# famoreno/stereo-vo

Hardware: AMD Instinct MI355X
Metric: stereo pairs/sec @1280×960 (higher is better)
Workload: dtype u8/f64

## Files before the change

### stereo_vo_amd/csrc/k_detect.hip

```cpp
#include <algorithm>
#include "svo_device.h"
#include "svo_kernels.h"
#include "../../include/svo_orb_tables.h"

__constant__ int c_umax[16];
__device__ __attribute__((aligned(16))) float4 g_brief_patf[SVO_BRIEF_NPAIRS];
__device__ __attribute__((aligned(16))) uint4 g_blur_gh[3 * 64], g_blur_gv[3 * 64];
#define SVO_DISC_E 256
__device__ uint32_t g_disc_m[SVO_DISC_E], g_disc_x[SVO_DISC_E];
#define DP_REACH SVO_BRIEF_REACH
#define DP_BW (2 * DP_REACH + 1)
#define DP_RW (DP_BW + 6)
#define DP_X0 (DP_REACH + 5)

hipError_t svo_upload_tables()
{
    hipError_t e = hipMemcpyToSymbol(HIP_SYMBOL(c_umax), svo_umax, sizeof(svo_umax));
    if (e != hipSuccess) return e;
    {
        static float4 pf[SVO_BRIEF_NPAIRS];
        for (int i = 0; i < SVO_BRIEF_NPAIRS; i++) pf[i] = make_float4((float)svo_brief_pat[i][0], (float)svo_brief_pat[i][2], (float)svo_brief_pat[i][1], (float)svo_brief_pat[i][3]);
        e = hipMemcpyToSymbol(HIP_SYMBOL(g_brief_patf), pf, sizeof(pf));
        if (e != hipSuccess) return e;
    }
// ... 346 lines not shown
#pragma unroll
        for (int g = 0; g < FT_ROWS; g++) {
            const uint32_t Cp = col[(g + 3) * (FT_LW / 4)], C = cc[g + 3], Cn = col[(g + 3) * (FT_LW / 4) + 2], N = cc[g], S = cc[g + 6];
            const uint32_t Eo = __builtin_amdgcn_alignbyte(Cn, C, 3), Wo = __builtin_amdgcn_alignbyte(C, Cp, 1);
            const uint32_t Ee = __builtin_amdgcn_alignbyte(Cn, C, 2);
            pe[g] = quick_half(C << 8, N << 8, Ee, S << 8, Cp, t2h);
            po[g] = quick_half(C, N, Eo, S, Wo, t2h);
        }
    }
    auto entry_of = [&](int b) -> int { return e_base + ((b & 7) << 6) + (b >> 3); };
    uint32_t m_left = 0;
    {
        const uint32_t one2 = 0x00010001u;
        uint32_t me = 0, mo = 0;
#pragma unroll
        for (int g = FT_ROWS - 1; g >= 0; g--) {
            uint32_t fe, fo;
            asm("v_pk_min_u16 %0, %1, %2" : "=v"(fe) : "v"(pe[g]), "s"(one2));
            asm("v_pk_min_u16 %0, %1, %2" : "=v"(fo) : "v"(po[g]), "s"(one2));
            if (g == FT_ROWS - 1) { me = fe; mo = fo; }
            else {
                asm("v_lshl_or_b32 %0, %1, 1, %2" : "=v"(me) : "v"(me), "v"(fe));
                asm("v_lshl_or_b32 %0, %1, 1, %2" : "=v"(mo) : "v"(mo), "v"(fo));
            }
        }
        uint32_t m = me | (mo << 8);
        const int cnt = __popc(m), inc = wave_inclusive_scan(cnt);
        const int total = __builtin_amdgcn_readlane(inc, 63);
        if (total) {
            unsigned wbase = 0;
            if ((tid & 63) == 0) wbase = atomicAdd(&s_count, (unsigned)total);
            unsigned idx = (unsigned)__builtin_amdgcn_readfirstlane((int)wbase) + (unsigned)(inc - cnt);
            while (m && idx < FT_LIST_CAP) {
                const int b = __builtin_ctz(m); m &= m - 1;
                list[idx++] = (unsigned short)entry_of(b);
            }
            m_left = m;
        }
    }
    __syncthreads();
    const int ns_all = (int)s_count, ns = min(ns_all, FT_LIST_CAP);
    const bool overflow = ns_all > FT_LIST_CAP;
    if (c.debug_mode == 2) return;
    auto win_off = [&](int e) -> int { return (e >> 6) * FT_LW + (e & 63) + (3 * FT_LW + 4); };
    for (int i = tid; i < ns; i += FT_NT) {
        const int e = list[i];
        score[e] = (uint8_t)fast_score_lds(tile, win_off(e), th_fast);
    }
    if (__builtin_expect(overflow, 0)) {
        for (uint32_t m = m_left; m; m &= m - 1) {
            const int e = entry_of(__builtin_ctz(m));
            score[e] = (uint8_t)fast_score_lds(tile, win_off(e), th_fast);
        }
    }
    __syncthreads();
    if (c.debug_mode == 3) return;
    auto nms_round = [&](bool has, int e) {
        bool keep = false; uint32_t key = 0;
        if (has) {
            const int r = e >> 6, q = e & 63;
            const int nb = e - FT_SP - 1; int nbm = nb; asm volatile("" : "+v"(nbm));
            const int v = score[nbm + FT_SP + 1];
            const int n0 = score[nb], n1 = score[nbm + 1], n2 = score[nb + 2], n3 = score[nb + FT_SP], n4 = score[nb + FT_SP + 2];
            const int n5 = score[nb + 2 * FT_SP], n6 = score[nbm + 2 * FT_SP + 1], n7 = score[nb + 2 * FT_SP + 2];
            const int mx = max(max(max(n0, n1), max(n2, n3)), max(max(n4, n5), max(n6, n7)));
            const int x = x0 - 1 + q, y = y0 - 1 + r;
            keep = (v > mx) & (r >= 1) & (r <= FT_H) & (q >= 1) & (q <= FT_W) & (x < gw - SVO_EDGE) & (y < gh - SVO_EDGE);
            key = ((uint32_t)v << 24) | (0xFFFFFFu - (uint32_t)(y * gw + x));
        }
        const unsigned long long m = __ballot(keep);
        if (m) {
            unsigned b2 = 0;
            const int leader = __ffsll((long long)m) - 1;
            if ((tid & 63) == leader) b2 = atomicAdd(&s_nout, (unsigned)__popcll(m));
            b2 = __shfl(b2, leader, 64);
            if (keep) out_keys[b2 + __popcll(m & ((1ull << (tid & 63)) - 1ull))] = key;
        }
    };
    for (int base = 0; base < ns; base += FT_NT) {
        const int i = base + tid;
        nms_round(i < ns, i < ns ? (int)list[i] : 0);
    }
    if (__builtin_expect(overflow, 0)) {
        uint32_t m = m_left;
        while (__ballot(m != 0)) {
            const bool has = m != 0;
            const int e = has ? entry_of(__builtin_ctz(m)) : 0;
            m &= m - 1;
            nms_round(has, e);
        }
    }
    __syncthreads();
    if (tid < 64) {
        const unsigned nout = s_nout;
        if (nout != 0 && c.debug_mode != 4) {
            const LevelGeom& g = c.lv[level];
            unsigned gbase = 0;
            if (tid == 0) gbase = atomicAdd(&c.cand_cnt[(img * SVO_MAX_LEVELS + level) * SVO_CNT_STRIDE], nout);
            gbase = __shfl(gbase, 0, 64);
            uint32_t* dst = c.cand_keys + (long long)img * c.cand_total + g.cand_off;
            for (unsigned i = tid; i < nout; i += 64) {
                if (gbase + i < (unsigned)g.cand_cap) dst[gbase + i] = out_keys[i];
                else raise_detect_status(c, img >> 1, SVO_ST_CAND_OVERFLOW);
            }
        }
    }
}

__global__ void __launch_bounds__(FT_NT) __attribute__((amdgpu_waves_per_eu(8, 8))) k_fast(DevCtx c)
{
    SVO_TL_SCOPE(c, TL_FAST, 0);
    __shared__ FastSmem sm;
    const uint32_t slot = blockIdx.x >> 3;
    const uint32_t work = c.debug_mode == 8 ? blockIdx.x : (((slot / FT_CHUNK) * 8 + (blockIdx.x & 7)) * FT_CHUNK + slot % FT_CHUNK);
    const int img = (int)fastdiv(work, c.div_tiles), tile_id = (int)work - img * c.n_tiles;
    if (img >= c.n_img) return;
    const uint4 e = c.fast_tiles[tile_id];
    const uint4 tha = ((const uint4*)(c.fast_th_used + img * SVO_MAX_LEVELS))[0], thb = ((const uint4*)(c.fast_th_used + img * SVO_MAX_LEVELS))[1];
    const uint8_t* base0 = c.img0[img];
    const int level = (int)(e.z & 0xFFu);
    const uint32_t thv[8] = { tha.x, tha.y, tha.z, tha.w, thb.x, thb.y, thb.z, thb.w };
    uint32_t th = thv[0];
#pragma unroll
    for (int l = 1; l < SVO_MAX_LEVELS; l++) th = level == l ? thv[l] : th;
    const uint8_t* src = level == 0 ? base0 : c.pyr + (long long)img * c.pyr_bytes + e.w;
    const int pitch = level == 0 ? c.img0_pitch : (int)(e.z >> 8);
    fast_tile(c, sm, img, level, src, pitch, (int)(e.y & 0xFFFFu), (int)(e.y >> 16), (int)(e.x & 0xFFFFu), (int)(e.x >> 16), (int)th);
}

__global__ void __launch_bounds__(FT_NT) k_fast_redo(DevCtx c)
{
    SVO_TL_SCOPE(c, TL_FAST, 1);
    __shared__ FastSmem sm;
    const unsigned n = *c.redo_n;
    if (n == 0) return;
    int first = (int)blockIdx.x;
    for (unsigned e = 0; e < n; e++) {
        const uint32_t il = c.redo_list[e];
        const int img = (int)(il / SVO_MAX_LEVELS), level = (int)(il % SVO_MAX_LEVELS);
        const int nt = c.lv[level].tiles_x * c.lv[level].tiles_y;
        int t = first;
        int pitch; const uint8_t* src = level_ptr(c, img, level, pitch);
        const int tx = c.lv[level].tiles_x, gw = c.lv[level].w, gh = c.lv[level].h;
        for (; t < nt; t += (int)gridDim.x) {
            const int by = t / tx, bx = t - by * tx;
            fast_tile(c, sm, img, level, src, pitch, gw, gh, SVO_EDGE + bx * FT_W, SVO_EDGE + by * FT_H, c.fast_th);
            __syncthreads();
        }
        first = t - nt;
    }
}


__device__ __forceinline__ float harris_at(const uint8_t* img, int pitch, int x, int y)
{
    int a = 0, b = 0, cc = 0;
    for (int dy = -3; dy <= 3; dy++) {
        const uint8_t* pm = img + (long long)(y + dy - 1) * pitch + x, *p0 = pm + pitch, *pp = p0 + pitch;
#pragma unroll
        for (int dx = -3; dx <= 3; dx++) {
            const int Ix = ((int)p0[dx + 1] - (int)p0[dx - 1]) * 2 + ((int)pm[dx + 1] - (int)pm[dx - 1]) + ((int)pp[dx + 1] - (int)pp[dx - 1]);
            const int Iy = ((int)pp[dx] - (int)pm[dx]) * 2 + ((int)pp[dx - 1] - (int)pm[dx - 1]) + ((int)pp[dx + 1] - (int)pm[dx + 1]);
            a += Ix * Ix; b += Iy * Iy; cc += Ix * Iy;
        }
    }
    const float s = 1.0f / (4.0f * 7.0f * 255.0f);
    const float s4 = s * s * s * s;
    const float fa = (float)a, fb = (float)b, fc = (float)cc;
    const float tr = fa + fb;
    return (fa * fb - fc * fc - 0.04f * tr * tr) * s4;
}

__device__ __forceinline__ float harris_at_dw(const uint8_t* img, int pitch, int x, int y)
{
    const int xa = (x - 4) & ~3, o = (x - 4) & 3;
    int px[9][9];
#pragma unroll
    for (int r = 0; r < 9; r++) {
        const uint3 pw = *(const uint3*)(img + (long long)(y - 4 + r) * pitch + xa);
        const uint32_t w0 = pw.x, w1 = pw.y, w2 = pw.z;
        const uint32_t A = __builtin_amdgcn_alignbyte(w1, w0, o), B = __builtin_amdgcn_alignbyte(w2, w1, o), C = w2 >> (8 * o);
#pragma unroll
        for (int k = 0; k < 4; k++) { px[r][k] = (A >> (8 * k)) & 0xFF; px[r][4 + k] = (B >> (8 * k)) & 0xFF; }
        px[r][8] = C & 0xFF;
    }
    int a = 0, b = 0, cc = 0;
#pragma unroll
    for (int r = 1; r < 8; r++) {
#pragma unroll
        for (int q = 1; q < 8; q++) {
            const int Ix = (px[r][q + 1] - px[r][q - 1]) * 2 + (px[r - 1][q + 1] - px[r - 1][q - 1]) + (px[r + 1][q + 1] - px[r + 1][q - 1]);
            const int Iy = (px[r + 1][q] - px[r - 1][q]) * 2 + (px[r + 1][q - 1] - px[r - 1][q - 1]) + (px[r + 1][q + 1] - px[r - 1][q + 1]);
            a += __mul24(Ix, Ix); b += __mul24(Iy, Iy); cc += __mul24(Ix, Iy);
        }
    }
    const float s = 1.0f / (4.0f * 7.0f * 255.0f);
    const float s4 = s * s * s * s;
    const float fa = (float)a, fb = (float)b, fc = (float)cc;
    const float tr = fa + fb;
    return (fa * fb - fc * fc - 0.04f * tr * tr) * s4;
}

template <int SEL_MAX>
__device__ __forceinline__ int select_block(const DevCtx& c, int redo_pass, int img, int level, unsigned long long* keys, uint32_t* sel, unsigned* hist, int* scan_s, unsigned* sv)
{
    constexpr int SEL_TIE_MAX = 2 * SEL_MAX;
    unsigned& s_prefix = sv[0]; unsigned& s_need = sv[1]; unsigned& s_sel = sv[2]; unsigned& s_tie = sv[3]; unsigned& s_ntie = sv[4];
    const LevelGeom& g = c.lv[level];
    const int tid = threadIdx.x;
    const int il = img * SVO_MAX_LEVELS + level;
    if (redo_pass && !c.redo_flag[il]) return 0;
    unsigned nc = c.cand_cnt[il * SVO_CNT_STRIDE];
    if (nc > (unsigned)g.cand_cap) nc = g.cand_cap;
    const unsigned K = min(nc, (unsigned)(2 * g.quota));
    const uint32_t th_used = c.fast_th_used[il], th_base = (uint32_t)c.fast_th;
    if (!redo_pass && g.quota > 0 && th_used > th_base && nc < (unsigned)(2 * g.quota)) {
        if (tid == 0) {
            c.redo_flag[il] = 1; c.redo_list[atomicAdd(c.redo_n, 1u)] = (uint32_t)il;
            atomicAdd(c.redo_n + 1, 1u);
            c.cand_cnt[il * SVO_CNT_STRIDE] = 0; c.fast_th_used[il] = th_base; c.fast_th_dyn[il] = 0;
        }
        return 0;
    }
    if (K == 0 || g.quota <= 0) { if (tid == 0) { c.lvl_n[il] = 0; c.sel_n[il] = 0; c.fast_th_dyn[il] = 0; } return 0; }
    const uint32_t* ck = c.cand_keys + (long long)img * c.cand_total + g.cand_off;
    uint32_t* tie = (uint32_t*)keys;
    for (int i = tid; i < 256; i += blockDim.x) hist[i] = 0;
    if (tid == 0) { s_sel = 0; s_tie = 0; }
    __syncthreads();
    for (unsigned base = tid; base < nc; base += 8 * 512) {
        uint32_t k[8];
#pragma unroll
        for (int u = 0; u < 8; u++) { const unsigned i = base + u * 512; k[u] = i < nc ? ck[i] : 0u; }
#pragma unroll
        for (int u = 0; u < 8; u++) if (base + u * 512 < nc) atomicAdd(&hist[k[u] >> 24], 1u);
    }
    __syncthreads();
    if (c.debug_mode == 31) return 0;
    unsigned prefix = 0, mask = 0, need = K;
    {
        const int mine = tid < 256 ? (int)hist[255 - tid] : 0;
        int tot;
        const int before = block_exclusive_scan(mine, scan_s, &tot);
        if (tid < 256 && (unsigned)before < need && need <= (unsigned)(before + mine)) { s_prefix = (unsigned)(255 - tid) << 24; s_need = need - (unsigned)before; s_ntie = (unsigned)mine; }
        const unsigned M = 3u * (unsigned)g.quota + 32u;
        if (tid < 256 && (unsigned)before < M && M <= (unsigned)(before + mine)) c.fast_th_dyn[il] = (uint32_t)(255 - tid) > th_base ? (uint32_t)(255 - tid) : 0u;
        if (tid == 0 && (unsigned)tot < M) {
            const unsigned dens = max(hist[min(th_used, 255u)], 1u), lower = (M - (unsigned)tot) / dens + 1u;
            c.fast_th_dyn[il] = th_used > th_base + lower ? th_used - lower : 0u;
        }
        __syncthreads();
        prefix = s_prefix; need = s_need; mask = 0xFF000000u;
    }
    const unsigned n_tie = s_ntie;
    uint32_t cutoff;
    const unsigned K_ties = (K - need) + n_tie;
    if (K_ties <= (unsigned)SEL_MAX) {
        cutoff = prefix;
        for (unsigned base = tid; base < nc; base += 8 * 512) {
            uint32_t k[8];
#pragma unroll
            for (int u = 0; u < 8; u++) { const unsigned i = base + u * 512; k[u] = i < nc ? ck[i] : 0u; }
#pragma unroll
            for (int u = 0; u < 8; u++) if (base + u * 512 < nc && k[u] >= cutoff) sel[atomicAdd(&s_sel, 1u)] = k[u];
        }
        __syncthreads();
        return (int)K_ties;
    }
    if (tid == 0) raise_detect_status(c, img >> 1, SVO_ST_CAND_OVERFLOW);
    if (n_tie <= SEL_TIE_MAX) {
        for (unsigned base = tid; base < nc; base += 8 * 512) {
            uint32_t k[8];
#pragma unroll
            for (int u = 0; u < 8; u++) { const unsigned i = base + u * 512; k[u] = i < nc ? ck[i] : 0u; }
#pragma unroll
            for (int u = 0; u < 8; u++) {
                if (base + u * 512 >= nc) continue;
                if ((k[u] & 0xFF000000u) > prefix) sel[atomicAdd(&s_sel, 1u)] = k[u];
                else if ((k[u] & 0xFF000000u) == prefix) tie[atomicAdd(&s_tie, 1u)] = k[u];
            }
        }
        __syncthreads();
        for (int shift = 16; shift >= 0; shift -= 8) {
            for (int i = tid; i < 256; i += blockDim.x) hist[i] = 0;
            __syncthreads();
            for (unsigned i = tid; i < n_tie; i += blockDim.x) { const uint32_t k = tie[i]; if ((k & mask) == prefix) atomicAdd(&hist[(k >> shift) & 255u], 1u); }
            __syncthreads();
            const int mine = tid < 256 ? (int)hist[255 - tid] : 0;
            int tot;
            const int before = block_exclusive_scan(mine, scan_s, &tot);
            if (tid < 256 && (unsigned)before < need && need <= (unsigned)(before + mine)) { s_prefix = prefix | ((unsigned)(255 - tid) << shift); s_need = need - (unsigned)before; }
            __syncthreads();
            prefix = s_prefix; need = s_need; mask |= 255u << shift;
            __syncthreads();
        }
        cutoff = prefix;
        for (unsigned i = tid; i < n_tie; i += blockDim.x) { const uint32_t k = tie[i]; if (k >= cutoff) sel[atomicAdd(&s_sel, 1u)] = k; }
        __syncthreads();
    } else {
        for (int shift = 16; shift >= 0; shift -= 8) {
            for (int i = tid; i < 256; i += blockDim.x) hist[i] = 0;
            __syncthreads();
            for (unsigned i = tid; i < nc; i += blockDim.x) { const uint32_t k = ck[i]; if ((k & mask) == prefix) atomicAdd(&hist[(k >> shift) & 255u], 1u); }
            __syncthreads();
            const int mine = tid < 256 ? (int)hist[255 - tid] : 0;
            int tot;
            const int before = block_exclusive_scan(mine, scan_s, &tot);
            if (tid < 256 && (unsigned)before < need && need <= (unsigned)(before + mine)) { s_prefix = prefix | ((unsigned)(255 - tid) << shift); s_need = need - (unsigned)before; }
            __syncthreads();
            prefix = s_prefix; need = s_need; mask |= 255u << shift;
            __syncthreads();
        }
        cutoff = prefix;
        for (unsigned i = tid; i < nc; i += blockDim.x) { const uint32_t k = ck[i]; if (k >= cutoff) { const unsigned sl = atomicAdd(&s_sel, 1u); if (sl < SEL_MAX) sel[sl] = k; } }
        __syncthreads();
    }
    return (int)K;
}

template <int SEL_MAX>
__global__ void __launch_bounds__(512) k_select(DevCtx c, int redo_pass)
{
    SVO_TL_SCOPE(c, TL_SELECT, redo_pass);
    __shared__ unsigned long long keys[SEL_MAX];
    __shared__ uint32_t sel[SEL_MAX];
    __shared__ unsigned hist[256];
    __shared__ int scan_s[32];
    __shared__ unsigned sv[5];
    const int level = blockIdx.y, img = blockIdx.x, tid = threadIdx.x;
    const int K = select_block<SEL_MAX>(c, redo_pass, img, level, keys, sel, hist, scan_s, sv);
    if (K <= 0) return;
    uint32_t* gsel = c.sel_keys + ((long long)img * SVO_MAX_LEVELS + level) * c.sel_max;
    for (int i = tid; i < K; i += blockDim.x) gsel[i] = sel[i];
    if (tid == 0) c.sel_n[img * SVO_MAX_LEVELS + level] = K;
}

__global__ void __launch_bounds__(256) k_harris(DevCtx c)
{
    SVO_TL_SCOPE(c, TL_HARRIS, 0);
    const int img = blockIdx.x, level = blockIdx.z, i = blockIdx.y * 256 + threadIdx.x;
    const LevelGeom& g = c.lv[level];
    const int K = g.quota > 0 ? c.sel_n[img * SVO_MAX_LEVELS + level] : 0;
    if ((int)(blockIdx.y * 256) >= K) return;
    if (i >= K) return;
    const long long o = ((long long)img * SVO_MAX_LEVELS + level) * c.sel_max + i;
    const uint32_t pos = 0xFFFFFFu - (c.sel_keys[o] & 0xFFFFFFu);
    const int x = (int)(pos % (uint32_t)g.w), y = (int)(pos / (uint32_t)g.w);
    int pitch; const uint8_t* lim = level_ptr(c, img, level, pitch);
    const bool aligned = (((uintptr_t)lim | (uintptr_t)pitch) & 3) == 0;
    const float r = aligned ? harris_at_dw(lim, pitch, x, y) : harris_at(lim, pitch, x, y);
    c.sel_resp[o] = ((unsigned long long)ord32(r) << 32) | (unsigned long long)(0xFFFFFFFFu - pos);
}

#define SS_NB 1024
template <int SEL_MAX>
__device__ __forceinline__ void rank_block(const DevCtx& c, int img, int level, int K, const unsigned long long (&mykey)[SEL_MAX / 512],
                                           unsigned long long* keys, unsigned long long* tmp, int* cnt, int* off, int* scan_s, unsigned* sv)
{
    unsigned& s_mn = sv[0]; unsigned& s_mx = sv[1]; unsigned& s_mnp = sv[2]; int& s_np = *(int*)(sv + 3);
    const int tid = threadIdx.x;
    const LevelGeom& g = c.lv[level];
    if (tid == 0) { s_mn = 0xFFFFFFFFu; s_mx = 0u; s_mnp = 0xFFFFFFFFu; s_np = 0; }
    for (int i = tid; i < SS_NB; i += blockDim.x) cnt[i] = 0;
    __syncthreads();
    int mypos[SEL_MAX / 512], myb[SEL_MAX / 512];
    unsigned lmn = 0xFFFFFFFFu, lmx = 0u, lmnp = 0xFFFFFFFFu; int lnp = 0;
#pragma unroll
    for (int it = 0; it < SEL_MAX / 512; it++) {
        const int i = tid + it * 512;
        if (i < K) {
            const unsigned h = (unsigned)(mykey[it] >> 32);
            lmn = min(lmn, h); lmx = max(lmx, h);
            if (h >= 0x80000000u) { lmnp = min(lmnp, h); lnp++; }
        }
    }
#pragma unroll
    for (int o = 32; o > 0; o >>= 1) {
        lmn = min(lmn, (unsigned)__shfl_xor((int)lmn, o, 64)); lmx = max(lmx, (unsigned)__shfl_xor((int)lmx, o, 64));
        lmnp = min(lmnp, (unsigned)__shfl_xor((int)lmnp, o, 64)); lnp += __shfl_xor(lnp, o, 64);
    }
    if (c.debug_mode == 41) return;
    if ((tid & 63) == 0) { atomicMin(&s_mn, lmn); atomicMax(&s_mx, lmx); atomicMin(&s_mnp, lmnp); atomicAdd(&s_np, lnp); }
    __syncthreads();
    const unsigned mn = s_np >= g.quota ? s_mnp : s_mn;
    const float scale = (float)(SS_NB - 1) / ((float)(s_mx - mn) + 1.0f);
#pragma unroll
    for (int it = 0; it < SEL_MAX / 512; it++) {
        const int i = tid + it * 512;
        if (i < K) {
            const unsigned h = (unsigned)(mykey[it] >> 32);
            const int b = h < mn ? SS_NB - 1 : SS_NB - 1 - min((int)((float)(h - mn) * scale), SS_NB - 1);
            myb[it] = b; mypos[it] = atomicAdd(&cnt[b], 1);
        }
    }
    __syncthreads();
    if (c.debug_mode == 42) return;
    int run = 0;
    for (int base = 0; base < SS_NB; base += 512) {
        int tot;
        const int o = block_exclusive_scan(cnt[base + tid], scan_s, &tot);
        off[base + tid] = run + o;
        run += tot;
        __syncthreads();
    }
    if (c.debug_mode == 43) return;
#pragma unroll
    for (int it = 0; it < SEL_MAX / 512; it++) { const int i = tid + it * 512; if (i < K) tmp[off[myb[it]] + mypos[it]] = mykey[it]; }
    __syncthreads();
    if (c.debug_mode == 44) return;
#pragma unroll
    for (int it = 0; it < SEL_MAX / 512; it++) {
        const int i = tid + it * 512;
        if (i < K) {
            const int b0 = off[myb[it]], nb = cnt[myb[it]];
            if (b0 >= min(K, g.quota)) continue;
            int greater = 0;
            for (int q = 0; q < nb; q++) greater += tmp[b0 + q] > mykey[it] ? 1 : 0;
            keys[b0 + greater] = mykey[it];
        }
    }
    __syncthreads();
    if (c.debug_mode == 45) return;
    const int nout = min(K, g.quota);
    for (int i = tid; i < nout; i += blockDim.x) {
        const unsigned long long k = keys[i];
        const uint32_t pos = 0xFFFFFFFFu - (uint32_t)(k & 0xFFFFFFFFull);
        c.lvl_pos[(long long)img * c.raw_cap + g.slot_off + i] = (pos % (uint32_t)g.w) | ((pos / (uint32_t)g.w) << 16);
        c.lvl_resp[(long long)img * c.raw_cap + g.slot_off + i] = inv_ord32((uint32_t)(k >> 32));
    }
    if (tid == 0) c.lvl_n[img * SVO_MAX_LEVELS + level] = nout;
}


template <int SEL_MAX>
__global__ void __launch_bounds__(512) k_select_sort(DevCtx c)
{
    SVO_TL_SCOPE(c, TL_SELECT_SORT, 0);
    extern __shared__ __attribute__((aligned(16))) unsigned char ss_smem[];
    unsigned long long* keys = (unsigned long long*)ss_smem, *tmp = keys + SEL_MAX;
    __shared__ int cnt[SS_NB], off[SS_NB], scan_s[32];
    __shared__ unsigned sv[4];
    const int level = blockIdx.y, img = blockIdx.x, tid = threadIdx.x;
    if (c.lv[level].quota <= 0) return;
    const int K = c.sel_n[img * SVO_MAX_LEVELS + level];
    if (K <= 0) return;
    const unsigned long long* gk = c.sel_resp + ((long long)img * SVO_MAX_LEVELS + level) * c.sel_max;
    unsigned long long mykey[SEL_MAX / 512];
#pragma unroll
    for (int it = 0; it < SEL_MAX / 512; it++) { const int i = tid + it * 512; mykey[it] = i < K ? gk[i] : 0ull; }
    rank_block<SEL_MAX>(c, img, level, K, mykey, keys, tmp, cnt, off, scan_s, sv);
}


#define DP_PW 12
#define DP_LROWS 48
typedef int dp_v4i __attribute__((ext_vector_type(4)));

__device__ __forceinline__ float atan2_deg(float y, float x)
{
    const float p1 = 57.283627f, p3 = -18.667446f, p5 = 8.9140005f, p7 = -2.5397246f;
    const float ax = fabsf(x), ay = fabsf(y);
    const bool steep = !(ax >= ay);
    const float cq = (steep ? ax : ay) / ((steep ? ay : ax) + 2.220446e-16f);
    const float c2 = cq * cq;
    float a = (((p7 * c2 + p5) * c2 + p3) * c2 + p1) * cq;
    if (steep) a = 90.0f - a;
    if (x < 0.0f) a = 180.0f - a;
    if (y < 0.0f) a = 360.0f - a;
    return a;
}

__device__ __forceinline__ void sincos_f32(float x, float& sn, float& cs)
{
    const int k = (int)(x * 0.63661977f + 0.5f);
    const float fk = (float)k;
    const float r = ((x - fk * 1.5703125f) - fk * 4.837512969970703125e-4f) - fk * 7.54978995489188216e-8f;
    const float z = r * r;
    const float sp = ((-1.9515295891e-4f * z + 8.3321608736e-3f) * z - 1.6666654611e-1f) * z * r + r;
    const float cp = ((2.443315711809948e-5f * z - 1.388731625493765e-3f) * z + 4.166664568298827e-2f) * z * z - 0.5f * z + 1.0f;
    const bool odd = k & 1;
    const float s0 = odd ? cp : sp, c0 = odd ? sp : cp;
    sn = (k & 2) ? -s0 : s0;
    cs = (((k + 1) & 2) != 0) ? -c0 : c0;
}

__device__ __forceinline__ uint32_t udot4(uint32_t a, uint32_t b, uint32_t acc)
{
    return __builtin_amdgcn_udot4(a, b, acc, false);
}

template <int NW, bool TL>
__global__ void __launch_bounds__(NW * 64) k_describe(DevCtx c, FastDiv gx_div, int pre, int kpw)
{
    SVO_TL_SCOPE(c, TL_DESCRIBE, pre);
    __shared__ __attribute__((aligned(16))) uint32_t raw32[NW][2][DP_LROWS * DP_PW + 4];
    __shared__ __attribute__((aligned(16))) float4 s_pat[SVO_BRIEF_NPAIRS];
    __shared__ uint32_t s_disc_m[SVO_DISC_E], s_disc_x[SVO_DISC_E];
    static_assert(NW * 64 == SVO_BRIEF_NPAIRS && NW * 64 == SVO_DISC_E, "one table entry per thread");
    __shared__ __attribute__((aligned(16))) uint4 s_gh[TL ? 3 * 64 : 1], s_gv[TL ? 3 * 64 : 1];
    s_pat[threadIdx.x] = g_brief_patf[threadIdx.x]; s_disc_m[threadIdx.x] = g_disc_m[threadIdx.x]; s_disc_x[threadIdx.x] = g_disc_x[threadIdx.x];
    if (TL && threadIdx.x < 3 * 64) { s_gh[threadIdx.x] = g_blur_gh[threadIdx.x]; s_gv[threadIdx.x] = g_blur_gv[threadIdx.x]; }
    __syncthreads();
    const int wid = __builtin_amdgcn_readfirstlane((int)(threadIdx.x >> 6)), lane = threadIdx.x & 63;
// ... 870 lines not shown
```

### stereo_vo_amd/csrc/svo_device.h

```cpp
#pragma once
#include <hip/hip_runtime.h>
#include <stdint.h>
#include "../../include/svo_hip.h"

#define SVO_EDGE 31
#define SVO_RANSAC_HYP 1000
#define SVO_RANSAC_PAD 1024
#define SVO_RANSAC_REG 16
#define SVO_RANSAC_RSLOTS 48
#define SVO_RANSAC_SLOTS (SVO_RANSAC_PAD / SVO_RANSAC_REG * SVO_RANSAC_RSLOTS)
#define SVO_RANSAC_CHUNK0 32
#define SVO_RANSAC_FEW 320
#ifndef SVO_RANSAC_CHUNK1
#define SVO_RANSAC_CHUNK1 160
#endif
#define SVO_SEL_MAX 2048
#define SVO_FT_W 62
#define SVO_FT_H 62
#define SVO_CNT_STRIDE 32
#define SVO_RS_ATT 1152
#define SVO_RS_SMALL_N 64
#define SVO_RS_ATT_SMALL 11008
#define SVO_LMEDS_MAX_N 14
#define SVO_LMEDS_ITERS 300
// ... 9 lines not shown
static inline FastDiv make_fastdiv(uint32_t d)
{
    FastDiv f; f.d = d;
    uint32_t l = 0; while ((1ull << l) < d) l++;
    f.m = (uint32_t)((((1ull << l) - d) << 32) / d + 1);
    f.s1 = l < 1 ? l : 1; f.s2 = l > 1 ? l - 1 : 0;
    return f;
}
#ifdef __HIPCC__
__device__ __forceinline__ uint32_t fastdiv(uint32_t x, const FastDiv& f)
{
    const uint32_t t = __umulhi(f.m, x);
    return (t + ((x - t) >> f.s1)) >> f.s2;
}
#endif

struct LevelGeom {
    int w, h, pitch;
    int tiles_x, tiles_y, tile_off;
    int quota, slot_off;
    int cand_cap, cand_off;
    long long offset;
    float scale;
    int rtab_off;
};

struct LaneState {
    int prev_slot;
    int has_prev;
    int has_cur;
    int m_error;
    double last_pose[6];
    unsigned it_counter;
    int reset_ids;
    int last_match_id;
    int last_kf_max_id;
    int num_tracked_last_kf;
    int pad;
};

struct DevCtx {
    int n_lanes, n_img, n_levels;
    int W, H;
    int oct_cap, n_oct;
    int ow[SVO_MAX_OCTAVES], oh[SVO_MAX_OCTAVES];
    int kps_to_detect[SVO_MAX_OCTAVES];
    int fast_orb;
    int max_h;
    int img0_pitch;
    int max_kps, raw_cap, cand_total, n_tiles, n_slots;
    int sel_max;
    uint8_t* big_scratch;
    uint8_t* gn_scratch;
    FastDiv div_tiles;
    int fast_th, orb_th;
    int debug_mode;
    long long pyr_bytes;
    LevelGeom lv[SVO_MAX_LEVELS];
    const uint8_t** img0;
    uint8_t* pyr;
    int* rtab;
    uint32_t* cand_keys;
    uint32_t* cand_cnt;
    uint32_t* fast_th_dyn;
    uint32_t* fast_th_used;
    const uint4* fast_tiles;
    uint32_t* redo_flag;
    uint32_t* redo_list;
    uint32_t* redo_n;
    uint32_t* lvl_pos;
    float* lvl_resp;
    uint32_t* sel_keys;
    unsigned long long* sel_resp;
    int* sel_n;
    int* lvl_n;
    svo_keypoint* raw_kps;
    uint8_t* raw_desc;
    int* raw_n;
    uint2* desc_work;
    int* desc_n;
    svo_keypoint* kps;
    uint8_t* desc;
    int* final_slot;
    uint8_t* mdesc;
    int* n_kps;
    svo_dmatch* matches;
    int* n_matches;
    int* row_index;
    int* mrow_index;
    int* ids;
    int* n_ids;
    int* bf_idx;
    int* bf_dist;
    int* trk_kq;
    int* trk_nk;
    float* trk_pts;
    double* rs_F;
    double* rs_guard;
    int* rs_cnt;
    int* rs_k;
    int* rs_nvalid;
    int* rs_bound;
    int* rs_gen;
    const unsigned short* rs_att;
    int rs_att_nmax;
    const unsigned long long* rs_att_state;
    int rs_c1;
    int rs_c0;
    unsigned short* rs_smp;
    int* rs_sched;
    int* rs_ticket;
    int* rs_floor;
    svo_index_pair* tracked;
    int* n_tracked;
    double* gn_lmk;
    float* gn_obs;
    double* residual;
    int* outliers;
    svo_stereo_camera* cams;
    LaneState* lane;
    svo_result* results;
    uint32_t* status;
    uint32_t* det_status;
    int det_ahead;
    int rest_prio;
    struct TlRec* tl;
    int tl_step;
    int tl_pad;
};

struct TlRec { unsigned long long t0, t1; };
#define SVO_TL_STEPS 16
#define SVO_TL_SUB 128
enum { TL_BEGIN = 0, TL_RESIZE, TL_FAST, TL_SELECT, TL_HARRIS, TL_SELECT_SORT, TL_NMS, TL_DESCRIBE, TL_HAMMING, TL_LR_FILTER, TL_TRK_FILTER,
       TL_RS_SCHED, TL_RS_HYP, TL_RS_COUNT, TL_TRK_FINAL, TL_MATCH_IDS, TL_GN, TL_OTHER, TL_KINDS };

#ifdef __HIPCC__
#define SVO_LATENCY_CHAIN(c) do { if ((c).rest_prio == 3) __builtin_amdgcn_s_setprio(3); else if ((c).rest_prio == 2) __builtin_amdgcn_s_setprio(2); else if ((c).rest_prio == 1) __builtin_amdgcn_s_setprio(1); } while (0)
#endif

#ifdef __HIPCC__
struct TlScope {
    TlRec* base; unsigned long long t0;
    __device__ __forceinline__ TlScope(const DevCtx& c, int kind, int aux) : base(nullptr), t0(0)
    {
        if (c.tl) {
            base = c.tl + ((((size_t)(c.tl_step & (SVO_TL_STEPS - 1)) << 8) | (size_t)((kind & 31) << 3) | (size_t)(aux & 7)) << 7);
            t0 = wall_clock64();
        }
    }
    __device__ __forceinline__ ~TlScope()
    {
        if (base) {
            const unsigned g = gridDim.x, stride = g > 32u ? g / 32u : 1u, wave = threadIdx.x >> 6, nw = (blockDim.x + 63u) >> 6;
            int sub = -1;
            if (wave == 0u && blockIdx.x + 1u == g) sub = 63;
            else if (wave == 0u && blockIdx.x % stride == 0u) sub = (int)min(blockIdx.x / stride, 62u);
            else if (g <= 64u && wave + 1u == nw) sub = 64 + (int)blockIdx.x;
            const unsigned long long act = __ballot(1);
            if (sub >= 0 && (int)(threadIdx.x & 63u) == __ffsll((long long)act) - 1) *(ulonglong2*)(base + sub) = make_ulonglong2(t0, (unsigned long long)wall_clock64());
        }
    }
};
#define SVO_TL_SCOPE(c, kind, aux) TlScope _tl_scope((c), (kind), (aux))
#endif

__device__ __forceinline__ void raise_detect_status(const DevCtx& c, int lane, uint32_t bit)
{
    if (c.det_ahead) { atomicOr(&c.det_status[lane], bit); return; }
    atomicOr(&c.status[lane], bit); atomicOr(&c.results[lane].status, (int)bit);
}

__device__ __forceinline__ const uint8_t* level_ptr(const DevCtx& c, int img, int level, int& pitch)
{
    if (level == 0) { pitch = c.img0_pitch; return c.img0[img]; }
    pitch = c.lv[level].pitch;
    return c.pyr + (long long)img * c.pyr_bytes + c.lv[level].offset;
}

__device__ __forceinline__ long long feat_base(const DevCtx& c, int vl, int slot, int side)
{
    return (((long long)vl * 2 + slot) * 2 + side) * c.max_kps;
}
__device__ __forceinline__ int feat_cnt_idx(int lane, int slot, int side) { return (lane * 2 + slot) * 2 + side; }
__device__ __forceinline__ long long match_base(const DevCtx& c, int lane, int slot) { return ((long long)lane * 2 + slot) * c.max_kps; }

__device__ __forceinline__ uint32_t ord32(float f)
{
    uint32_t u = __float_as_uint(f);
    return (u & 0x80000000u) ? ~u : (u | 0x80000000u);
}
__device__ __forceinline__ float inv_ord32(uint32_t k)
{
    uint32_t u = (k & 0x80000000u) ? (k & 0x7FFFFFFFu) : ~k;
    return __uint_as_float(u);
}

__device__ __forceinline__ void wave_lds_sync()
{
    __builtin_amdgcn_fence(__ATOMIC_RELEASE, "workgroup");
    __builtin_amdgcn_wave_barrier();
    __builtin_amdgcn_fence(__ATOMIC_ACQUIRE, "workgroup");
}

template <bool DESC>
__device__ __forceinline__ void bitonic_sort_lds(unsigned long long* keys, int P)
{
    const int tid = threadIdx.x, nt = blockDim.x, half = P >> 1;
    __syncthreads();
    for (int k = 2; k <= P; k <<= 1) {
        for (int j = k >> 1; j > 0; j >>= 1) {
            if (j >= 128 || (j == 64 && k >= 256)) __syncthreads(); else wave_lds_sync();
            for (int t = tid; t < half; t += nt) {
                const int i = ((t & ~(j - 1)) << 1) | (t & (j - 1)), ixj = i | j;
                const unsigned long long a = keys[i], b = keys[ixj];
                const bool up = ((i & k) == 0);
                const bool lt = a < b;
                const bool sw = DESC ? (lt == up) : (lt != up);
                if (sw) { keys[i] = b; keys[ixj] = a; }
            }
        }
    }
    __syncthreads();
}

__device__ __forceinline__ int wave_sum_uniform(int v)
{
    v += __builtin_amdgcn_update_dpp(0, v, 0xB1, 0xF, 0xF, false);
    v += __builtin_amdgcn_update_dpp(0, v, 0x4E, 0xF, 0xF, false);
    v += __builtin_amdgcn_update_dpp(0, v, 0x141, 0xF, 0xF, false);
    v += __builtin_amdgcn_update_dpp(0, v, 0x140, 0xF, 0xF, false);
    return __builtin_amdgcn_readlane(v, 0) + __builtin_amdgcn_readlane(v, 16) + __builtin_amdgcn_readlane(v, 32) + __builtin_amdgcn_readlane(v, 48);
}

__device__ __forceinline__ int wave_reduce_sum_i32(int v)
{
#pragma unroll
    for (int o = 32; o > 0; o >>= 1) v += __shfl_xor(v, o, 64);
    return v;
}
__device__ __forceinline__ double wave_reduce_sum_f64(double v)
{
#pragma unroll
    for (int o = 32; o > 0; o >>= 1) v += __shfl_xor(v, o, 64);
    return v;
}

__device__ __forceinline__ int wave_inclusive_scan(int v)
{
    v += __builtin_amdgcn_update_dpp(0, v, 0x111, 0xF, 0xF, true);
    v += __builtin_amdgcn_update_dpp(0, v, 0x112, 0xF, 0xF, true);
    v += __builtin_amdgcn_update_dpp(0, v, 0x114, 0xF, 0xF, true);
    v += __builtin_amdgcn_update_dpp(0, v, 0x118, 0xF, 0xF, true);
    v += __builtin_amdgcn_update_dpp(0, v, 0x142, 0xA, 0xF, false);
    v += __builtin_amdgcn_update_dpp(0, v, 0x143, 0xC, 0xF, false);
    return v;
}

__device__ __forceinline__ int block_exclusive_scan(int v, int* scratch, int* total)
{
    const int lane = threadIdx.x & 63, wid = __builtin_amdgcn_readfirstlane((int)(threadIdx.x >> 6)), nw = (blockDim.x + 63) >> 6;
    const int inc = wave_inclusive_scan(v);
    __syncthreads();
    if (lane == 63) scratch[wid] = inc;
    __syncthreads();
    const int t = lane < nw ? scratch[lane] : 0;
    *total = wave_sum_uniform(t);
    const int base = wave_sum_uniform(lane < wid ? t : 0);
    return base + inc - v;
}

#define SVO_NMS_UNDECIDED 2
__device__ __forceinline__ uint32_t nms_hash_slot(uint32_t key, int HSZ) { return ((key * 2654435761u) >> 7) & (uint32_t)(HSZ - 1); }

__device__ __forceinline__ uint32_t nms_lookup(const uint32_t* hkey, const uint32_t* hval, int HSZ, uint32_t key)
{
    uint32_t h = nms_hash_slot(key, HSZ);
    for (;;) {
        const uint32_t k = hkey[h];
        if (k == key) return hval[h];
        if (k == 0xFFFFFFFFu) return 0xFFFFFFFFu;
        h = (h + 1) & (uint32_t)(HSZ - 1);
    }
}

template <int ITEMS>
__device__ __forceinline__ void grid_nms_block(int n, unsigned gly, const uint32_t* cellxy, uint32_t* hkey, uint32_t* hval, int HSZ,
                                               volatile unsigned char* state, volatile int* flag)
{
    const int tid = threadIdx.x, nt = blockDim.x;
    for (int i = tid; i < HSZ; i += nt) { hkey[i] = 0xFFFFFFFFu; hval[i] = 0xFFFFFFFFu; }
    __syncthreads();
    for (int i = tid; i < n; i += nt) {
        const uint32_t c = cellxy[i];
        if (c == 0xFFFFFFFFu) continue;
        const uint32_t key = (c >> 16) * gly + (c & 0xFFFFu);
        uint32_t h = nms_hash_slot(key, HSZ);
        for (;;) {
            const uint32_t old = atomicCAS(&hkey[h], 0xFFFFFFFFu, key);
            if (old == 0xFFFFFFFFu || old == key) { atomicMin(&hval[h], (uint32_t)i); break; }
            h = (h + 1) & (uint32_t)(HSZ - 1);
        }
    }
    __syncthreads();
    for (int i = tid; i < n; i += nt) {
        const uint32_t c = cellxy[i];
        unsigned char st = 0;
        if (c != 0xFFFFFFFFu && nms_lookup(hkey, hval, HSZ, (c >> 16) * gly + (c & 0xFFFFu)) == (uint32_t)i) st = SVO_NMS_UNDECIDED;
        state[i] = st;
    }
    __syncthreads();
// ... 74 lines not shown
```

Baseline: 74410.

## Rewrite Harris response with packed int16 separable Sobel and sdot2 accumulation

```diff
diff --git a/stereo_vo_amd/csrc/k_detect.hip b/stereo_vo_amd/csrc/k_detect.hip
--- a/stereo_vo_amd/csrc/k_detect.hip
+++ b/stereo_vo_amd/csrc/k_detect.hip
@@ -522,47 +522,65 @@
 }
 
 
-__device__ __forceinline__ float harris_at(const uint8_t* img, int pitch, int x, int y)
-{
+typedef short i16x2 __attribute__((ext_vector_type(2)));
+struct HarrisRow { i16x2 d[4], s[4]; };
+
+__device__ __forceinline__ i16x2 px_pair(uint32_t hi, uint32_t lo, uint32_t sel) { return __builtin_bit_cast(i16x2, __builtin_amdgcn_perm(hi, lo, sel)); }
+
+__device__ __forceinline__ void harris_row(uint32_t A, uint32_t B, uint32_t C, i16x2 two, HarrisRow& o)
+{
+    const i16x2 p01 = px_pair(0u, A, 0x0c010c00u), p12 = px_pair(0u, A, 0x0c020c01u), p23 = px_pair(0u, A, 0x0c030c02u), p34 = px_pair(B, A, 0x0c040c03u);
+    const i16x2 p45 = px_pair(0u, B, 0x0c010c00u), p56 = px_pair(0u, B, 0x0c020c01u), p67 = px_pair(0u, B, 0x0c030c02u);
+    const i16x2 p6z = px_pair(0u, B, 0x0c0c0c02u), p7z = px_pair(0u, B, 0x0c0c0c03u), p8z = px_pair(0u, C, 0x0c0c0c00u);
+    o.d[0] = p23 - p01; o.d[1] = p45 - p23; o.d[2] = p67 - p45; o.d[3] = p8z - p6z;
+    o.s[0] = p12 * two + p01 + p23; o.s[1] = p34 * two + p23 + p45; o.s[2] = p56 * two + p45 + p67; o.s[3] = p7z * two + p6z + p8z;
+}
+
+typedef const __attribute__((address_space(1))) uint8_t* harris_gptr;
+typedef uint32_t u32x3 __attribute__((ext_vector_type(3)));
+
+__device__ __forceinline__ u32x3 harris_load_dw(harris_gptr row, uint32_t off) { return *(const __attribute__((address_space(1))) u32x3*)(row + off); }
+
+__device__ __forceinline__ u32x3 harris_load_bytes(harris_gptr row, uint32_t off)
+{
+    harris_gptr p = row + off;
+    u32x3 v;
+    v.x = (uint32_t)p[0] | ((uint32_t)p[1] << 8) | ((uint32_t)p[2] << 16) | ((uint32_t)p[3] << 24);
+    v.y = (uint32_t)p[4] | ((uint32_t)p[5] << 8) | ((uint32_t)p[6] << 16) | ((uint32_t)p[7] << 24);
+    v.z = (uint32_t)p[8];
+    return v;
+}
+
+#define HARRIS_AHEAD 4
+
+template <bool ALIGNED>
+__device__ __forceinline__ float harris_response(const uint8_t* img, int pitch, int x, int y)
+{
+    HarrisRow w[3];
+    u32x3 ld[9];
+    uint32_t two_bits = 0x00020002u;
+    asm volatile("" : "+s"(two_bits));
+    const i16x2 two = __builtin_bit_cast(i16x2, two_bits);
     int a = 0, b = 0, cc = 0;
-    for (int dy = -3; dy <= 3; dy++) {
-        const uint8_t* pm = img + (long long)(y + dy - 1) * pitch + x, *p0 = pm + pitch, *pp = p0 + pitch;
-#pragma unroll
-        for (int dx = -3; dx <= 3; dx++) {
-            const int Ix = ((int)p0[dx + 1] - (int)p0[dx - 1]) * 2 + ((int)pm[dx + 1] - (int)pm[dx - 1]) + ((int)pp[dx + 1] - (int)pp[dx - 1]);
-            const int Iy = ((int)pp[dx] - (int)pm[dx]) * 2 + ((int)pp[dx - 1] - (int)pm[dx - 1]) + ((int)pp[dx + 1] - (int)pm[dx + 1]);
-            a += Ix * Ix; b += Iy * Iy; cc += Ix * Iy;
-        }
-    }
-    const float s = 1.0f / (4.0f * 7.0f * 255.0f);
-    const float s4 = s * s * s * s;
-    const float fa = (float)a, fb = (float)b, fc = (float)cc;
-    const float tr = fa + fb;
-    return (fa * fb - fc * fc - 0.04f * tr * tr) * s4;
-}
-
-__device__ __forceinline__ float harris_at_dw(const uint8_t* img, int pitch, int x, int y)
-{
-    const int xa = (x - 4) & ~3, o = (x - 4) & 3;
-    int px[9][9];
-#pragma unroll
-    for (int r = 0; r < 9; r++) {
-        const uint3 pw = *(const uint3*)(img + (long long)(y - 4 + r) * pitch + xa);
-        const uint32_t w0 = pw.x, w1 = pw.y, w2 = pw.z;
-        const uint32_t A = __builtin_amdgcn_alignbyte(w1, w0, o), B = __builtin_amdgcn_alignbyte(w2, w1, o), C = w2 >> (8 * o);
-#pragma unroll
-        for (int k = 0; k < 4; k++) { px[r][k] = (A >> (8 * k)) & 0xFF; px[r][4 + k] = (B >> (8 * k)) & 0xFF; }
-        px[r][8] = C & 0xFF;
-    }
-    int a = 0, b = 0, cc = 0;
-#pragma unroll
-    for (int r = 1; r < 8; r++) {
-#pragma unroll
-        for (int q = 1; q < 8; q++) {
-            const int Ix = (px[r][q + 1] - px[r][q - 1]) * 2 + (px[r - 1][q + 1] - px[r - 1][q - 1]) + (px[r + 1][q + 1] - px[r + 1][q - 1]);
-            const int Iy = (px[r + 1][q] - px[r - 1][q]) * 2 + (px[r + 1][q - 1] - px[r - 1][q - 1]) + (px[r + 1][q + 1] - px[r - 1][q + 1]);
-            a += __mul24(Ix, Ix); b += __mul24(Iy, Iy); cc += __mul24(Ix, Iy);
-        }
+    const int o = (x - 4) & 3;
+    uint32_t off = (uint32_t)(y - 4) * (uint32_t)pitch + (uint32_t)(ALIGNED ? (x - 4) & ~3 : x - 4);
+    harris_gptr row = (harris_gptr)img;
+#pragma unroll
+    for (int r = 0; r < HARRIS_AHEAD; r++, row += pitch) ld[r] = ALIGNED ? harris_load_dw(row, off) : harris_load_bytes(row, off);
+#pragma unroll
+    for (int r = 0; r < 9; r++, row += pitch) {
+        if (r + HARRIS_AHEAD < 9) ld[r + HARRIS_AHEAD] = ALIGNED ? harris_load_dw(row, off) : harris_load_bytes(row, off);
+        if (ALIGNED) harris_row(__builtin_amdgcn_alignbyte(ld[r].y, ld[r].x, o), __builtin_amdgcn_alignbyte(ld[r].z, ld[r].y, o), ld[r].z >> (8 * o), two, w[r % 3]);
+        else harris_row(ld[r].x, ld[r].y, ld[r].z, two, w[r % 3]);
+        if (r >= 2) {
+            const HarrisRow& up = w[(r - 2) % 3], & mid = w[(r - 1) % 3], & dn = w[r % 3];
+#pragma unroll
+            for (int k = 0; k < 4; k++) {
+                const i16x2 Ix = mid.d[k] * two + up.d[k] + dn.d[k], Iy = dn.s[k] - up.s[k];
+                a = __builtin_amdgcn_sdot2(Ix, Ix, a, false); b = __builtin_amdgcn_sdot2(Iy, Iy, b, false); cc = __builtin_amdgcn_sdot2(Ix, Iy, cc, false);
+            }
+        }
+        asm volatile("" : "+v"(off), "+v"(a), "+v"(b), "+v"(cc));
     }
     const float s = 1.0f / (4.0f * 7.0f * 255.0f);
     const float s4 = s * s * s * s;
@@ -705,7 +723,7 @@
     if (tid == 0) c.sel_n[img * SVO_MAX_LEVELS + level] = K;
 }
 
-__global__ void __launch_bounds__(256) k_harris(DevCtx c)
+__global__ void __launch_bounds__(256) __attribute__((amdgpu_waves_per_eu(8, 8))) k_harris(DevCtx c)
 {
     SVO_TL_SCOPE(c, TL_HARRIS, 0);
     const int img = blockIdx.x, level = blockIdx.z, i = blockIdx.y * 256 + threadIdx.x;
@@ -718,7 +736,7 @@
     const int x = (int)(pos % (uint32_t)g.w), y = (int)(pos / (uint32_t)g.w);
     int pitch; const uint8_t* lim = level_ptr(c, img, level, pitch);
     const bool aligned = (((uintptr_t)lim | (uintptr_t)pitch) & 3) == 0;
-    const float r = aligned ? harris_at_dw(lim, pitch, x, y) : harris_at(lim, pitch, x, y);
+    const float r = aligned ? harris_response<true>(lim, pitch, x, y) : harris_response<false>(lim, pitch, x, y);
     c.sel_resp[o] = ((unsigned long long)ord32(r) << 32) | (unsigned long long)(0xFFFFFFFFu - pos);
 }
 
diff --git a/stereo_vo_amd/csrc/svo_device.h b/stereo_vo_amd/csrc/svo_device.h
--- a/stereo_vo_amd/csrc/svo_device.h
+++ b/stereo_vo_amd/csrc/svo_device.h
@@ -185,11 +185,12 @@
     __device__ __forceinline__ ~TlScope()
     {
         if (base) {
-            const unsigned g = gridDim.x, stride = g > 32u ? g / 32u : 1u, wave = threadIdx.x >> 6, nw = (blockDim.x + 63u) >> 6;
+            const unsigned g = gridDim.x * gridDim.y * gridDim.z, bid = blockIdx.x + gridDim.x * (blockIdx.y + gridDim.y * blockIdx.z);
+            const unsigned stride = g > 32u ? g / 32u : 1u, wave = threadIdx.x >> 6, nw = (blockDim.x + 63u) >> 6;
             int sub = -1;
-            if (wave == 0u && blockIdx.x + 1u == g) sub = 63;
-            else if (wave == 0u && blockIdx.x % stride == 0u) sub = (int)min(blockIdx.x / stride, 62u);
-            else if (g <= 64u && wave + 1u == nw) sub = 64 + (int)blockIdx.x;
+            if (wave == 0u && bid + 1u == g) sub = 63;
+            else if (wave == 0u && bid % stride == 0u) sub = (int)min(bid / stride, 62u);
+            else if (g <= 64u && wave + 1u == nw) sub = 64 + (int)bid;
             const unsigned long long act = __ballot(1);
             if (sub >= 0 && (int)(threadIdx.x & 63u) == __ffsll((long long)act) - 1) *(ulonglong2*)(base + sub) = make_ulonglong2(t0, (unsigned long long)wall_clock64());
         }
```

New measurement: 74750 (median of 6 runs). No clear change (+0.5%).
